# mmbajo/PROBA-V

Measured on AMD Instinct MI355X. Metric: LR-patches/sec fwd+bwd (WDSR-B r12 t9, 16x16, bs128), higher is better.
Workload: dtype f32 (products as 3 scaled-fp16-piece MFMA products, f32 accumulate)

## Files before the change

### proba-v_amd/csrc/kernels_cw4.hip

```cpp
#include "kernels_x6.h"
#include "x6_device.h"
#include <cstdlib>
#include <algorithm>

namespace probav {
#ifdef CW4_DIAG
namespace diag {
#endif

struct Cw4Args {
    ConvGeom g;
    int Wp, Wt, nsplit, SR, nstrips, nslot;
    unsigned mTo, mNvr, mTi, mNslot;
};

namespace {
__device__ __forceinline__ int qdiv(int v, int d, unsigned m) { return (int)__umulhi((unsigned)v, m) + (d == 1 ? v : 0); }
unsigned qmagic(int d) { return d <= 1 ? 0u : (unsigned)((0x100000000ull + (unsigned)d - 1) / (unsigned)d); }
typedef float f32x4u __attribute__((ext_vector_type(4), aligned(4)));
typedef unsigned u32x4b __attribute__((ext_vector_type(4)));
constexpr int CW4_PSE = 151;
constexpr int CW4_PS = 16 * CW4_PSE;
constexpr int CW4_ROW = 8 * CW4_PS;
constexpr unsigned CW4_OOB = 0x40000000u;
}

#ifdef CW4_STAMP
__device__ unsigned long long g_cw4_stamps[1024 * 8];
#endif

#define CW4_SBAR() __builtin_amdgcn_sched_barrier(0)
#ifdef CW4_STAMP
#define CW4_ST(k) do { unsigned long long t_; asm volatile("s_memtime %0\n\ts_waitcnt lgkmcnt(0)" : "=s"(t_) :: "memory"); st_acc[k] += t_ - st_prev; st_prev = t_; } while (0)
#ifdef CW4_STAMP_ROUNDS
#define CW4_STR(k) CW4_ST(k)
#else
#define CW4_STR(k) do { } while (0)
#endif
#else
#define CW4_STR(k) do { } while (0)
#define CW4_ST(k) do { } while (0)
#endif

template <int CIN, int COUT, int TP, bool RELU, bool SKIP, bool BIAS>
__global__ __launch_bounds__(256, 1) void conv3_w4_kernel(Cw4Args a, const float* __restrict__ x, const uint4* __restrict__ wfrag, const float* __restrict__ bias,
                                                         const float* __restrict__ skip, float* __restrict__ y, Amax am)
{
    extern __shared__ __attribute__((aligned(16))) unsigned char lds[];
    constexpr int NST = CIN == 25 ? 5 : 6, KB = 9 * NST, G = 3 * KB;
    constexpr int NW1R = CIN == 25 ? 12 : 8;
    constexpr int NCH = CIN == 25 ? 3 : 4;
    constexpr int PS = CW4_PS, ROW = CW4_ROW;
    constexpr int PD = 2;
    constexpr int TO = TP - 2;
    const ConvGeom& g = a.g;
    const int tid = threadIdx.x, lane = tid & 63, half = lane >> 5, col = lane & 31;
    const int wave = __builtin_amdgcn_readfirstlane(tid >> 6);
    const int per = a.nstrips * a.nsplit;
    const int n = blockIdx.x / per, srem = blockIdx.x - n * per;
    const int strip = srem / a.nsplit, sp = srem - strip * a.nsplit;
    const int ws0 = sp * a.Wt, hb = strip * a.SR;
    const int SRr = g.Ho - hb < a.SR ? g.Ho - hb : a.SR;
    const int nvr = a.Wt * g.To, NV = SRr * nvr, NTL = (NV + 31) >> 5, nround = (NTL + 3) >> 2;
    const int NS = a.nslot;
    float omax = 0.f;
#ifdef CW4_STAMP
    unsigned long long st_t0 = __builtin_amdgcn_s_memtime(), st_r0 = __builtin_amdgcn_s_memrealtime();
    unsigned long long st_prev = st_t0, st_acc[8] = {0, 0, 0, 0, 0, 0, 0, 0};
#endif

    const int lw0 = a.nsplit == 1 ? g.pw : 0, Wl = a.nsplit == 1 ? g.Wi : a.Wt + 2;
    const int nvs = Wl * g.Ti, items = nvs * NCH;
    const int ea = h3_exp(am.x[n]);
    const float sa = pow2i(ea);
    int s_srcb[2], s_offb[2];
    float s_sc[2];
    int s3_o[3], s3_offb = 0;
    float s3_sc[3] = {0.f, 0.f, 0.f};
    {
        auto locate = [&](int lv, int& lw, int& t, int& iwc, int& colok) {
            const int lwr = qdiv(lv, g.Ti, a.mTi);
            t = lv - lwr * g.Ti; lw = lw0 + lwr;
            const int iw = ws0 + lw - g.pw;
            colok = (iw >= 0 ? 1 : 0) & (iw < g.Wi ? 1 : 0);
            iwc = iw < 0 ? 0 : (iw < g.Wi ? iw : g.Wi - 1);
        };
#pragma unroll
        for (int k = 0; k < 2; ++k) {
            const int it = tid + 256 * k;
            const int ic = it < items ? it : items - 1;
            const int lv = CIN == 25 ? (int)(((unsigned)ic * 43691u) >> 17) : ic >> 2;
            const int cc = ic - lv * NCH;
            int lw, t, iwc, colok;
            locate(lv, lw, t, iwc, colok);
            s_srcb[k] = ((iwc * g.Ti + t) * CIN + 8 * cc) * 4;
            s_offb[k] = (lw * TO + t) * 16 + cc * PS;
            s_sc[k] = colok ? sa : 0.f;
        }
        if constexpr (CIN == 25) {
            const int lv = tid < nvs ? tid : nvs - 1;
            int lw, t, iwc, colok;
            locate(lv, lw, t, iwc, colok);
            const int base = ((iwc * g.Ti + t) * CIN + 24) * 4;
            s3_offb = (lw * TO + t) * 16 + 3 * PS;
            const int ok3[3] = {colok && t - 1 >= 0, colok, colok && t + 1 < g.Ti};
#pragma unroll
            for (int j = 0; j < 3; ++j) { s3_o[j] = base + (ok3[j] ? (j - 1) * CIN * 4 : 0); s3_sc[j] = ok3[j] ? sa : 0.f; }
        }
    }
    const long xsample = (long)g.Hi * g.Wi * g.Ti * CIN;
    const __amdgpu_buffer_rsrc_t xrs = __builtin_amdgcn_make_buffer_rsrc(const_cast<float*>(x + (long)n * xsample), 0, (unsigned)xsample * 4u, 0x00020000);
    const int xrowb = g.Wi * g.Ti * CIN * 4;
    struct Staged { u32x4b v[2][2]; unsigned g3[3]; };
    auto row_of = [&](int q, int& rowoff, float& rokf) {
        const int ih = hb - g.ph + q;
        const bool rok = ih >= 0 && ih < g.Hi;
        rowoff = (rok ? ih : 0) * xrowb;
        rokf = rok ? 1.f : 0.f;
    };
    auto stage_load_items = [&](int rowoff, Staged& sv) {
#pragma unroll
        for (int k = 0; k < 2; ++k) {
            sv.v[k][0] = __builtin_amdgcn_raw_buffer_load_b128(xrs, s_srcb[k], rowoff, 0);
            sv.v[k][1] = __builtin_amdgcn_raw_buffer_load_b128(xrs, s_srcb[k] + 16, rowoff, 0);
        }
    };
    auto stage_load_g3 = [&](int rowoff, Staged& sv) {
#ifdef CW4_ABL_NOG3
        sv.g3[0] = sv.g3[1] = sv.g3[2] = 0u; return;
#endif
        if constexpr (CIN == 25) {
#pragma unroll
            for (int j = 0; j < 3; ++j) sv.g3[j] = __builtin_amdgcn_raw_buffer_load_b32(xrs, s3_o[j], rowoff, 0);
        }
    };
    auto slot_of = [&](int q) -> int { return (q - qdiv(q, NS, a.mNslot) * NS) * ROW; };
    struct Cut { float sc[2], sg[3]; f32x2 t[4]; unsigned h0[4], h1[4]; float u[3]; };
    constexpr int ROW_MOPS = CIN == 25 ? 52 : 41;
    auto stage_mop = [&](int m, int slot, float rokf, Staged& sv, Cut& c, bool reload, int rel) {
        if (m < 5) {
            if (m < 2) c.sc[m] = s_sc[m] * rokf;
            else if (CIN == 25) c.sg[m - 2] = s3_sc[m - 2] * rokf;
            return;
        }
        m -= 5;
        if (m < 36) {
            const int k = m / 18, i = m % 18;
            if (i < 16) {
                const int p = i >> 2, op = i & 3;
                if (op == 0) {
                    const u32x4b q = sv.v[k][p >> 1];
                    const f32x2 v = {__uint_as_float(q[2 * (p & 1)]), __uint_as_float(q[2 * (p & 1) + 1])};
                    c.t[p] = v * (f32x2){c.sc[k], c.sc[k]};
                    if (p == 3 && reload) {
                        sv.v[k][0] = __builtin_amdgcn_raw_buffer_load_b128(xrs, s_srcb[k], rel, 0);
                        sv.v[k][1] = __builtin_amdgcn_raw_buffer_load_b128(xrs, s_srcb[k] + 16, rel, 0);
                    }
                } else if (op == 1) {
                    c.h0[p] = __builtin_bit_cast(unsigned, __builtin_convertvector(c.t[p], f16x2));
                } else if (op == 2) {
                    asm("v_fma_mixlo_f16 %0, %1, -1.0, %2 op_sel:[0,0,0] op_sel_hi:[1,0,0]" : "=v"(c.h1[p]) : "v"(c.h0[p]), "v"(c.t[p][0]));
                } else {
                    asm("v_fma_mixhi_f16 %0, %1, -1.0, %2 op_sel:[1,0,0] op_sel_hi:[1,0,0]" : "+v"(c.h1[p]) : "v"(c.h0[p]), "v"(c.t[p][1]));
                }
            } else {
#ifdef CW4_ABL_NOWRITE
                asm volatile("" :: "v"(c.h0[0]), "v"(c.h0[1]), "v"(c.h0[2]), "v"(c.h0[3]), "v"(c.h1[0]), "v"(c.h1[1]), "v"(c.h1[2]), "v"(c.h1[3]));
                return;
#endif
                unsigned char* ent = lds + slot + s_offb[k];
                if (i == 16) *reinterpret_cast<uint4*>(ent) = make_uint4(c.h0[0], c.h0[1], c.h0[2], c.h0[3]);
                else *reinterpret_cast<uint4*>(ent + 4 * PS) = make_uint4(c.h1[0], c.h1[1], c.h1[2], c.h1[3]);
            }
            return;
        }
        if constexpr (CIN == 25) {
            m -= 36;
            if (m < 3) { c.u[m] = __uint_as_float(sv.g3[m]) * c.sg[m]; if (m == 2 && reload) stage_load_g3(rel, sv); }
            else if (m == 3) c.h0[0] = __builtin_bit_cast(unsigned, __builtin_convertvector((f32x2){c.u[0], c.u[1]}, f16x2));
            else if (m == 4) c.h0[1] = __builtin_bit_cast(unsigned, __builtin_convertvector((f32x2){c.u[2], 0.f}, f16x2));
            else if (m == 5) asm("v_fma_mixlo_f16 %0, %1, -1.0, %2 op_sel:[0,0,0] op_sel_hi:[1,0,0]" : "=v"(c.h1[0]) : "v"(c.h0[0]), "v"(c.u[0]));
            else if (m == 6) asm("v_fma_mixhi_f16 %0, %1, -1.0, %2 op_sel:[1,0,0] op_sel_hi:[1,0,0]" : "+v"(c.h1[0]) : "v"(c.h0[0]), "v"(c.u[1]));
            else if (m == 7) c.h1[1] = 0u;
            else if (m == 8) asm("v_fma_mixlo_f16 %0, %1, -1.0, %2 op_sel:[0,0,0] op_sel_hi:[1,0,0]" : "+v"(c.h1[1]) : "v"(c.h0[1]), "v"(c.u[2]));
            else if (m == 9) *reinterpret_cast<uint2*>(lds + slot + s3_offb) = make_uint2(c.h0[0], c.h0[1]);
            else *reinterpret_cast<uint2*>(lds + slot + s3_offb + 4 * PS) = make_uint2(c.h1[0], c.h1[1]);
        }
    };
    auto need = [&](int r) -> int {
        const int vlast = (r + 1) * 128 - 1 < NV - 1 ? (r + 1) * 128 - 1 : NV - 1;
        return qdiv(vlast, nvr, a.mNvr) + 2;
    };

    CW4_ST(3);
    int hiq = nround > 0 ? need(0) : -1;
    Staged p0[4];
    int p0_slot[4];
    float p0_rok[4];
#pragma unroll
    for (int q = 0; q < 4; ++q) {
        int rowoff;
        row_of(q <= hiq ? q : 0, rowoff, p0_rok[q]);
        p0_slot[q] = slot_of(q <= hiq ? q : 0);
        stage_load_items(rowoff, p0[q]);
        stage_load_g3(rowoff, p0[q]);
    }
    constexpr int NQ = ((KB - NW1R) * 64 + 255) / 256;
    u32x4b w1q[NQ];
    const u32x4b* wfrag4 = reinterpret_cast<const u32x4b*>(wfrag);
    const int Z0c = a.Wp * (TP - 2);
    constexpr int NF = KB + NW1R, NF4 = (NF + 3) / 4;
    u32x4b xq[NF4];
#pragma unroll
    for (int i = 0; i < NF4; ++i) {
        int f = 4 * i + wave;
        f = f < NF ? f : NF - 1;
        xq[i] = wfrag4[(f < KB ? 2 * f : 2 * (f - KB) + 1) * 64 + lane];
    }
    const int tab = NS * ROW + (KB - NW1R) * 1024;
    const int tc = tid < g.Cout ? tid : 0;
    const unsigned tew = am.w[tc];
    const float tbv = (bias ? bias : reinterpret_cast<const float*>(am.w))[tc];
#pragma unroll
    for (int i = 0; i < NQ; ++i) {
        int e = tid + 256 * i;
        e = e < (KB - NW1R) * 64 ? e : (KB - NW1R) * 64 - 1;
        w1q[i] = wfrag4[(2 * (NW1R + (e >> 6)) + 1) * 64 + (e & 63)];
    }
    CW4_ST(4);
    if (tid < 32) {
        const int e = -(ea + h3_exp_w(tew));
        reinterpret_cast<int*>(lds + tab)[tid] = e;
        reinterpret_cast<float*>(lds + tab + 128)[tid] = (BIAS && bias && tid < g.Cout) ? ldexpf(tbv, -e) : 0.f;
    }
#pragma unroll
    for (int i = 0; i < NF4; ++i) {
        int f = 4 * i + wave;
        f = f < NF ? f : NF - 1;
        *reinterpret_cast<u32x4b*>(lds + f * 1024 + lane * 16) = xq[i];
    }
    asm volatile("s_waitcnt lgkmcnt(0)\n\ts_barrier" ::: "memory");
    f16x8 w0[KB], w1r[NW1R > 0 ? NW1R : 1];
#pragma unroll
    for (int K = 0; K < KB; ++K) { Frag f; f.u = *reinterpret_cast<const uint4*>(lds + K * 1024 + lane * 16); w0[K] = f.h; }
#pragma unroll
    for (int K = 0; K < NW1R; ++K) { Frag f; f.u = *reinterpret_cast<const uint4*>(lds + (KB + K) * 1024 + lane * 16); w1r[K] = f.h; }
#pragma unroll
    for (int K = 0; K < KB; ++K) asm volatile("" : "+a"(w0[K]));
#pragma unroll
    for (int K = 0; K < NW1R; ++K) asm volatile("" : "+a"(w1r[K]));
    asm volatile("s_waitcnt lgkmcnt(0)\n\ts_barrier" ::: "memory");
    if (a.nsplit == 1) {
        uint4* z = reinterpret_cast<uint4*>(lds);
        for (int i = tid; i < NS * ROW / 16; i += 256) z[i] = make_uint4(0u, 0u, 0u, 0u);
    } else {
        const int nzone = CW4_PSE - Z0c, nplanes = NS * 8;
        for (int i = tid; i < nzone * nplanes; i += 256) {
            const int pl = i / nzone, e = i - pl * nzone;
            *reinterpret_cast<uint4*>(lds + pl * PS + (Z0c + e) * 16) = make_uint4(0u, 0u, 0u, 0u);
        }
        if constexpr (CIN == 25) {
            for (int i = tid; i < Z0c * NS * 2; i += 256) {
                const int pl = i / Z0c, e = i - pl * Z0c;
                *reinterpret_cast<uint4*>(lds + (pl >> 1) * ROW + (3 + 4 * (pl & 1)) * PS + e * 16) = make_uint4(0u, 0u, 0u, 0u);
            }
        }
    }
    asm volatile("s_waitcnt lgkmcnt(0)\n\ts_barrier" ::: "memory");
    CW4_ST(5);
#pragma unroll
    for (int q = 0; q < 4; ++q) {
        Cut c;
#pragma unroll
        for (int m = 0; m < ROW_MOPS; ++m) stage_mop(m, p0_slot[q], p0_rok[q], p0[q], c, false, 0);
    }
    CW4_ST(6);
    const int w1a = NS * ROW + lane * 16;
#pragma unroll
    for (int i = 0; i < NQ; ++i) {
        int e = tid + 256 * i;
        e = e < (KB - NW1R) * 64 ? e : (KB - NW1R) * 64 - 1;
        *reinterpret_cast<u32x4b*>(lds + NS * ROW + e * 16) = w1q[i];
    }
    int eun[16];
    f32x16 bias16;
#pragma unroll
    for (int jj = 0; jj < 4; ++jj) {
        const int4 e4 = *reinterpret_cast<const int4*>(lds + tab + (8 * jj + 4 * half) * 4);
        const float4 b4 = *reinterpret_cast<const float4*>(lds + tab + 128 + (8 * jj + 4 * half) * 4);
        eun[4 * jj] = e4.x; eun[4 * jj + 1] = e4.y; eun[4 * jj + 2] = e4.z; eun[4 * jj + 3] = e4.w;
        bias16[4 * jj] = b4.x; bias16[4 * jj + 1] = b4.y; bias16[4 * jj + 2] = b4.z; bias16[4 * jj + 3] = b4.w;
    }
    const float lo = g.relu ? 0.f : -__builtin_inff();
    (void)lo;
    if (BIAS) asm volatile("" : "+a"(bias16));
    CW4_ST(7);
    asm volatile("s_waitcnt lgkmcnt(0)\n\ts_barrier" ::: "memory");

    const long out_base = ((long)n * g.Ho + hb) * g.Wo * g.To;
    const unsigned ybytes = (unsigned)(SRr * g.Wo * g.To * g.Cout) * 4u;
    const __amdgpu_buffer_rsrc_t yrs = __builtin_amdgcn_make_buffer_rsrc(y + out_base * g.Cout, 0, ybytes, 0x00020000);
    const __amdgpu_buffer_rsrc_t srs = __builtin_amdgcn_make_buffer_rsrc(const_cast<float*>(skip ? skip + out_base * g.Cout : y), 0, skip ? ybytes : 0u, 0x00020000);
    unsigned cofs[4];
#pragma unroll
    for (int jj = 0; jj < 4; ++jj) cofs[jj] = 8 * jj + 4 * half < COUT ? 4u * (8 * jj + 4 * half) : CW4_OOB;

    int offH[5];
    {
        const int pA[5] = {0, 2, 1, 0, 2}, pB[5] = {1, 0, 2, 1, 3};
#pragma unroll
        for (int st = 0; st < 5; ++st) offH[st] = (half ? pB[st] : pA[st]) * PS;
    }
    const int Z0 = a.Wp * TO;
    struct TileTmp { int vi, hrel, rem, w, t, x, e0, s0, s1, s2, b0, b1, b2, dlo, dhi; unsigned yo; };
    constexpr int TILE_STEPS = 14;
    auto tile_step = [&](int step, int tile, TileTmp& q, int (&bs)[9], unsigned (&eo)[4]) {
#define CW4_PIN(v) asm volatile("" : "+v"(v))
        if (step == 0) { const int v = tile * 32 + col; q.vi = v < NV ? v : NV - 1; q.yo = v < NV ? 0u : CW4_OOB; CW4_PIN(q.vi); CW4_PIN(q.yo); }
        if (step == 1) { q.hrel = (int)__umulhi((unsigned)q.vi, a.mNvr); q.rem = q.vi - q.hrel * nvr; CW4_PIN(q.hrel); CW4_PIN(q.rem); }
        if (step == 2) { q.w = (int)__umulhi((unsigned)q.rem, a.mTo); q.t = q.rem - q.w * g.To; CW4_PIN(q.w); CW4_PIN(q.t); }
        if (step == 3) { q.x = q.w * TO + q.t; q.s0 = q.hrel - (int)__umulhi((unsigned)q.hrel, a.mNslot) * NS; CW4_PIN(q.x); CW4_PIN(q.s0); }
        if (step == 4) { q.s1 = q.s0 + 1 < NS ? q.s0 + 1 : q.s0 + 1 - NS; q.e0 = q.x * 16 + (CIN == 32 ? half * PS : 0); CW4_PIN(q.s1); CW4_PIN(q.e0); }
        if (step == 5) { q.s2 = q.s1 + 1 < NS ? q.s1 + 1 : q.s1 + 1 - NS; CW4_PIN(q.s2); }
        if (step == 6) { q.b0 = q.s0 * ROW + q.e0; q.b1 = q.s1 * ROW + q.e0; q.b2 = q.s2 * ROW + q.e0; bs[1] = q.b0; bs[4] = q.b1; bs[7] = q.b2; CW4_PIN(bs[1]); CW4_PIN(bs[4]); CW4_PIN(bs[7]); }
        if (step == 7) { const int z = ((q.x - 1 - Z0) & 15) + Z0 - q.x; q.dlo = q.t == 0 ? z * 16 : -16; CW4_PIN(q.dlo); }
        if (step == 8) { const int z = ((q.x + 1 - Z0) & 15) + Z0 - q.x; q.dhi = q.t == TO - 1 ? z * 16 : 16; CW4_PIN(q.dhi); }
        if (step == 9) { bs[0] = q.b0 + q.dlo; bs[3] = q.b1 + q.dlo; bs[6] = q.b2 + q.dlo; CW4_PIN(bs[0]); CW4_PIN(bs[3]); CW4_PIN(bs[6]); }
        if (step == 10) { bs[2] = q.b0 + q.dhi; bs[5] = q.b1 + q.dhi; bs[8] = q.b2 + q.dhi; CW4_PIN(bs[2]); CW4_PIN(bs[5]); CW4_PIN(bs[8]); }
        if (step == 11) { q.yo += (unsigned)(((q.hrel * g.Wo + ws0 + q.w) * g.To + q.t) * COUT) * 4u; CW4_PIN(q.yo); }
        if (step == 12) { eo[0] = q.yo + cofs[0]; eo[1] = q.yo + cofs[1]; CW4_PIN(eo[0]); CW4_PIN(eo[1]); }
        if (step == 13) { eo[2] = q.yo + cofs[2]; eo[3] = q.yo + cofs[3]; CW4_PIN(eo[2]); CW4_PIN(eo[3]); }
#undef CW4_PIN
    };
    int adr5[5] = {0, 0, 0, 0, 0};
    auto read_A = [&](const int (&bs)[9], int K, Frag (&af)[2]) {
        const int gg = K / NST, st = K % NST, dh = gg / 3, dw = gg % 3;
        if constexpr (CIN == 25) {
            if (dw == 0) {
                const int bm = bs[3 * dh], bz = bs[3 * dh + 1], bp = bs[3 * dh + 2];
                const int b = st == 0 ? bm : st == 1 ? (half ? bz : bm) : st == 2 ? bz : st == 3 ? bp : (half ? bz : bp);
                adr5[st] = b + offH[st];
            }
            const unsigned char* p = lds + adr5[st];
            af[0].u = *reinterpret_cast<const uint4*>(p + dw * TO * 16);
            af[1].u = *reinterpret_cast<const uint4*>(p + dw * TO * 16 + 4 * PS);
        } else {
            const int d = st >> 1, kb = st & 1;
            const unsigned char* p = lds + bs[3 * dh + d];
            af[0].u = *reinterpret_cast<const uint4*>(p + dw * TO * 16 + 2 * kb * PS);
            af[1].u = *reinterpret_cast<const uint4*>(p + dw * TO * 16 + 2 * kb * PS + 4 * PS);
        }
    };
    auto read_W1 = [&](int K, Frag& wf) {
        if (K >= NW1R) wf.u = *reinterpret_cast<const uint4*>(lds + w1a + (K - NW1R) * 1024);
    };

    CW4_ST(2);
    f32x16 accA, accB;
#pragma unroll
    for (int i = 0; i < 16; ++i) { accA[i] = 0.f; accB[i] = 0.f; }
#ifdef CW4_ABL_2ACC
    f32x16 acc2;
    for (int i = 0; i < 16; ++i) acc2[i] = 0.f;
#endif
    f32x4u skq[4];
#pragma unroll
    for (int jj = 0; jj < 4; ++jj) skq[jj] = (f32x4u){0.f, 0.f, 0.f, 0.f};
    int bs[9];
    unsigned eo[4], eo_prev[4] = {CW4_OOB, CW4_OOB, CW4_OOB, CW4_OOB};
    {
        TileTmp q;
#pragma unroll
        for (int st = 0; st < TILE_STEPS; ++st) tile_step(st, wave, q, bs, eo);
    }
    Frag A[PD + 1][2], W1[PD + 1];
#pragma unroll
    for (int K = 0; K < PD; ++K) { read_A(bs, K, A[K]); read_W1(K, W1[K]); }

    Staged sv[2];
    auto round = [&](int r, f32x16& acc, f32x16& pacc) __attribute__((always_inline)) {
        const int hi_next = r + 1 < nround ? need(r + 1) : hiq;
        const int hi_nn = r + 2 < nround ? need(r + 2) : hi_next;
        const int q0 = hiq + 1, q1 = hi_next - hiq >= 2 ? hiq + 2 : hiq + 1;
        const int n0 = hi_next + 1, n1 = hi_nn - hi_next >= 2 ? hi_next + 2 : hi_next + 1;
        int rowoff[2], slot[2];
        float rokf[2], rokn;
        int dummy;
        row_of(q0, dummy, rokf[0]); row_of(q1, dummy, rokf[1]);
        row_of(n0, rowoff[0], rokn); row_of(n1, rowoff[1], rokn);
        slot[0] = slot_of(q0); slot[1] = slot_of(q1);
        Cut cut;
        TileTmp tq;
        int nbs[9];
        unsigned neo[4];
        float m2 = 0.f;
#pragma unroll
        for (int K = 0; K < KB; ++K) {
#pragma unroll
            for (int j = 0; j < 3; ++j) {
                const int gp = 3 * K + j;
                const int sl = K % (PD + 1);
                {
                    f16x8 wa;
                    if (j == 1) { if (K < NW1R) wa = w1r[K < NW1R ? K : 0]; else wa = W1[sl].h; }
                    else wa = w0[K];
                    const f16x8 xb = (j == 0) ? A[sl][1].h : A[sl][0].h;
                    if (gp == 0) {
                        if (BIAS) acc = __builtin_amdgcn_mfma_f32_32x32x16_f16(wa, xb, bias16, 0, 0, 0);
                        else {
                            f32x16 zero;
#pragma unroll
                            for (int i = 0; i < 16; ++i) zero[i] = 0.f;
                            acc = __builtin_amdgcn_mfma_f32_32x32x16_f16(wa, xb, zero, 0, 0, 0);
                        }
                    } else acc = __builtin_amdgcn_mfma_f32_32x32x16_f16(wa, xb, acc, 0, 0, 0);
                }
                CW4_SBAR();
#ifndef CW4_ABL_NOREAD
                if (j == 0) {
                    const int KN = K + PD, sn = KN % (PD + 1);
#ifndef CW4_ABL_W1LATE
                    read_W1(KN < KB ? KN : KN - KB, W1[sn]);
#endif
                    if (KN < KB) read_A(bs, KN, A[sn]); else read_A(nbs, KN - KB, A[sn]);
                }
#ifdef CW4_ABL_W1LATE
                if (j == 1) {
                    const int KN = K + PD, sn = KN % (PD + 1);
                    read_W1(KN < KB ? KN : KN - KB, W1[sn]);
                }
#endif
#endif
                if (K >= 1 && K <= 10 && j == 1) tile_step(K - 1, 4 * (r + 1) + wave, tq, nbs, neo);
                if (K >= 12 && K <= 15 && j == 1) tile_step(K - 2, 4 * (r + 1) + wave, tq, nbs, neo);
                if (K == 11 && j == 1) { CW4_STR(3); asm volatile("s_barrier" ::: "memory"); CW4_STR(4); }
#ifndef CW4_ABL_NOEPI
                if (K < 16 && j == 2) {
                    const int e = K, jj = e >> 2, i = e & 3;
                    float v = ldexpf(pacc[e], eun[e]);
                    if (RELU) v = relu_keep_nan(v, lo);
                    const float o = SKIP ? v + skq[jj][i] : v;
                    skq[jj][i] = o;
                    if ((e & 1) == 0) m2 = o; else asm volatile("v_max3_f32 %0, %0, |%1|, |%2|" : "+v"(omax) : "v"(m2), "v"(o));
                }
                if (j == 1 && (K == 4 || K == 8 || K == 12 || K == 16)) {
                    const int jj = K / 4 - 1;
                    const u32x4b o = {__float_as_uint(skq[jj][0]), __float_as_uint(skq[jj][1]), __float_as_uint(skq[jj][2]), __float_as_uint(skq[jj][3])};
                    if (COUT == 32 || jj < 3) __builtin_amdgcn_raw_buffer_store_b128(o, yrs, eo_prev[jj], 0, 0);
                    else __builtin_amdgcn_raw_buffer_store_b32(o[0], yrs, eo_prev[jj], 0, 0);
                    if (K == 16) omax = r == 0 ? 0.f : omax;
                }
                if (SKIP && (K == 17 || K == 18) && j > 0) {
                    const int jj = 2 * (K - 17) + j - 1;
                    if (COUT == 32 || jj < 3) {
                        const u32x4b q = __builtin_amdgcn_raw_buffer_load_b128(srs, eo[jj], 0, 0);
                        skq[jj] = (f32x4u){__uint_as_float(q[0]), __uint_as_float(q[1]), __uint_as_float(q[2]), __uint_as_float(q[3])};
                    } else {
                        const unsigned q = __builtin_amdgcn_raw_buffer_load_b32(srs, eo[jj], 0, 0);
                        skq[jj] = (f32x4u){__uint_as_float(q), 0.f, 0.f, 0.f};
                    }
                }
#endif
#ifndef CW4_ABL_NOSTAGE
                {
                    constexpr int NKS = (2 * ROW_MOPS + 5) / 6, KS0 = KB - PD - NKS;
                    if (K >= KS0 && K < KS0 + NKS && j > 0) {
                        const int m0 = (K - KS0) * 6 + 3 * (j - 1);
#pragma unroll
                        for (int m = m0; m < m0 + 3; ++m)
                            if (m < 2 * ROW_MOPS) {
#ifdef CW4_ABL_NOCUT
                                if (m == 0) asm volatile("" :: "v"(sv[0].v[0][0]), "v"(sv[0].v[1][1]), "v"(sv[1].v[0][0]), "v"(sv[1].v[1][1]));
                                continue;
#endif
                                stage_mop(m % ROW_MOPS, slot[m / ROW_MOPS], rokf[m / ROW_MOPS], sv[m / ROW_MOPS], cut, true, rowoff[m / ROW_MOPS]);
                            }
                    }
                }
#endif
                CW4_SBAR();
            }
        }
        CW4_STR(5);
#pragma unroll
        for (int d = 0; d < 9; ++d) bs[d] = nbs[d];
#pragma unroll
        for (int jj = 0; jj < 4; ++jj) { eo_prev[jj] = eo[jj]; eo[jj] = neo[jj]; }
        hiq = hi_next;
    };
    {
        const int hi1 = 1 < nround ? need(1) : hiq;
        const int n0 = hiq + 1, n1 = hi1 - hiq >= 2 ? hiq + 2 : hiq + 1;
        int ro;
        float rk;
        row_of(n0, ro, rk); stage_load_items(ro, sv[0]); stage_load_g3(ro, sv[0]);
        row_of(n1, ro, rk); stage_load_items(ro, sv[1]); stage_load_g3(ro, sv[1]);
    }
#pragma unroll 1
    for (int r = 0; r < nround; r += 2) {
        round(r, accA, accB);
        round(r + 1, accB, accA);
    }
    {
#pragma unroll
        for (int e = 0; e < 16; ++e) {
            const int jj = e >> 2, i = e & 3;
            float v = ldexpf(accB[e], eun[e]);
            if (RELU) v = relu_keep_nan(v, lo);
            const float o = SKIP ? v + skq[jj][i] : v;
            skq[jj][i] = o;
            omax = fmaxf(omax, fabsf(o));
        }
        if (nround == 0) omax = 0.f;
#pragma unroll
        for (int jj = 0; jj < 4; ++jj) {
            const u32x4b o = {__float_as_uint(skq[jj][0]), __float_as_uint(skq[jj][1]), __float_as_uint(skq[jj][2]), __float_as_uint(skq[jj][3])};
            if (COUT == 32 || jj < 3) __builtin_amdgcn_raw_buffer_store_b128(o, yrs, eo_prev[jj], 0, 0);
            else __builtin_amdgcn_raw_buffer_store_b32(o[0], yrs, eo_prev[jj], 0, 0);
        }
    }
#ifdef CW4_ABL_2ACC
    for (int i = 0; i < 16; ++i) omax += acc2[i];
#endif
    if (am.y) amax_commit(omax, am.y + n);
#ifdef CW4_STAMP
    if (lane == 0 && blockIdx.x < 256) {
        unsigned long long* o = g_cw4_stamps + (blockIdx.x * 4 + wave) * 8;
        o[0] = __builtin_amdgcn_s_memtime() - st_t0; o[1] = __builtin_amdgcn_s_memrealtime() - st_r0;
        for (int k = 2; k < 8; ++k) o[k] = st_acc[k];
    }
#endif
}

static bool cw4_plan(const ConvGeom& g, Cw4Args& p, size_t& lds_bytes, int& grid)
{
    if (g.kh != 3 || g.kw != 3 || g.kt != 3 || g.reflect_hw || g.reflect_t) return false;
    if (!((g.Cin == 25 && g.Cout == 32) || (g.Cin == 32 && (g.Cout == 25 || g.Cout == 32)))) return false;
    if (g.ph != 1 || g.pw != 1 || g.pt != 1) return false;
    if (g.Ho != g.Hi || g.Wo != g.Wi || g.To != g.Ti) return false;
    if (g.To != 9 && g.To != 7) return false;
    if (g.Ho < 3) return false;
    const int Tp = g.To + 2;
    for (int ns = 1; ns <= 4; ++ns) {
        if (g.Wo % ns) continue;
        const int wt = g.Wo / ns, nvr = wt * g.To;
        const int wp = wt + 2;
        const int nvs = (ns == 1 ? g.Wi : wt + 2) * g.Ti, items = nvs * (g.Cin == 25 ? 3 : 4);
        if (items > 512 || nvs > 256 || nvr < 64 || wp * g.To + 16 + 2 * g.To > CW4_PSE) continue;
        int nstrips = (256 + g.N * ns - 1) / (g.N * ns);
        if (nstrips < 1) nstrips = 1;
        if (nstrips > g.Ho / 4) nstrips = g.Ho / 4 > 0 ? g.Ho / 4 : 1;
        const int SR = (g.Ho + nstrips - 1) / nstrips;
        nstrips = (g.Ho + SR - 1) / SR;
        const int NV = SR * nvr, nround = ((NV + 31) / 32 + 3) / 4;
        auto needf = [&](int r) { const int vl = std::min(NV - 1, (r + 1) * 128 - 1); return vl / nvr + 2; };
        int nslot = needf(0) + 1;
        for (int r = 0; r + 1 < nround; ++r) nslot = std::max(nslot, needf(r + 1) - (r * 128) / nvr + 1);
        const int kb = g.Cin == 25 ? 45 : 54, nw1r = g.Cin == 25 ? 12 : 8;
        const size_t need = (size_t)nslot * CW4_ROW + (size_t)(kb - nw1r) * 1024 + 256;
        if (need > 163840) continue;
        p.g = g; p.Wp = wp; p.Wt = wt; p.nsplit = ns; p.SR = SR; p.nstrips = nstrips; p.nslot = nslot;
        p.mTo = qmagic(g.To); p.mNvr = qmagic(nvr); p.mTi = qmagic(g.Ti); p.mNslot = qmagic(nslot);
        lds_bytes = need; grid = g.N * nstrips * ns;
        return true;
    }
    return false;
}

bool cw4_conv_supported(const ConvGeom& g, bool gated)
{
    Cw4Args p;
    size_t lds_bytes;
    int grid;
    return !gated && cw4_plan(g, p, lds_bytes, grid);
}

bool cw4_conv_plan_ints(const ConvGeom& g, bool gated, int out[5])
{
    Cw4Args p;
    size_t lds_bytes;
    int grid;
    if (gated || !cw4_plan(g, p, lds_bytes, grid)) return false;
    out[0] = p.nsplit; out[1] = p.nstrips; out[2] = p.SR; out[3] = p.nslot; out[4] = grid;
    return true;
}

int cw4_conv_forward(const ConvGeom& g, const float* x, const float* wfrag, const float* bias, const float* skip, float* y, const Amax& am, hipStream_t s)
{
    Cw4Args p;
    size_t lds_bytes;
    int grid;
    if (!cw4_plan(g, p, lds_bytes, grid)) { set_error("cw4_conv_forward: unsupported geometry", hipSuccess); return PROBAV_EINVAL; }
    if (!am.x || !am.w) { set_error("cw4_conv_forward: H3 arithmetic needs the operands' amax slots", hipSuccess); return PROBAV_EINVAL; }
#define CW4_LAUNCH(C, O, T, R, S, B) return launch_lds<conv3_w4_kernel<C, O, T, R, S, B>>("conv3_w4", dim3(grid), dim3(256), lds_bytes, s, p, x, (const uint4*)wfrag, bias, skip, y, am)
#define CW4_LAUNCH_T(C, O) do { if (g.To == 9) CW4_LAUNCH(C, O, 11, true, true, true); else CW4_LAUNCH(C, O, 9, true, true, true); } while (0)
    if (g.Cin == 25 && g.To == 9 && !g.relu && skip && bias) CW4_LAUNCH(25, 32, 11, false, true, true);
    else if (g.Cin == 32 && g.Cout == 25 && g.To == 9 && !g.relu && !skip && !bias) CW4_LAUNCH(32, 25, 11, false, false, false);
    else if (g.Cin == 25) CW4_LAUNCH_T(25, 32);
    else if (g.Cout == 25) CW4_LAUNCH_T(32, 25);
    else CW4_LAUNCH_T(32, 32);
#undef CW4_LAUNCH_T
#undef CW4_LAUNCH
}

#ifdef CW4_DIAG
}
#endif
}
```

Baseline: 20620.

## Split leftover tail tiles' K reduction across waves in conv3 w4 kernel

When the last strip leaves one or two 32-voxel tiles beyond a multiple of four, those tiles are pulled out of the main round loop. They get a dedicated tail phase where the four waves split the K chain of MFMAs and reduce the partial accumulators through LDS. The aim is to stop a final round running with most waves idle on clamped, masked tiles. The cost is extra barriers, LDS exchange traffic and a duplicated epilogue, plus odd-round handling in the main loop.

```diff
diff --git a/proba-v_amd/csrc/kernels_cw4.hip b/proba-v_amd/csrc/kernels_cw4.hip
--- a/proba-v_amd/csrc/kernels_cw4.hip
+++ b/proba-v_amd/csrc/kernels_cw4.hip
@@ -2,6 +2,7 @@
 #include "x6_device.h"
 #include <cstdlib>
 #include <algorithm>
+#include <type_traits>
 
 namespace probav {
 #ifdef CW4_DIAG
@@ -61,7 +62,12 @@
     const int strip = srem / a.nsplit, sp = srem - strip * a.nsplit;
     const int ws0 = sp * a.Wt, hb = strip * a.SR;
     const int SRr = g.Ho - hb < a.SR ? g.Ho - hb : a.SR;
-    const int nvr = a.Wt * g.To, NV = SRr * nvr, NTL = (NV + 31) >> 5, nround = (NTL + 3) >> 2;
+    const int nvr = a.Wt * g.To, NV = SRr * nvr;
+    const int NVS = g.Ho * nvr, NTLS = (NVS + 31) >> 5;
+    const int ntail = (hb + SRr == g.Ho && ((NTLS & 3) == 1 || (NTLS & 3) == 2)) ? (NTLS & 3) : 0;
+    const int NVm = ntail ? NV - (NVS - 32 * (NTLS - ntail)) : NV;
+    const int NTL = (NVm + 31) >> 5, nmain = (NTL + 3) >> 2, nround = nmain + (ntail ? 1 : 0);
+    const int NVml = NVm > 0 ? NVm - 1 : 0;
     const int NS = a.nslot;
     float omax = 0.f;
 #ifdef CW4_STAMP
@@ -188,7 +194,7 @@
         }
     };
     auto need = [&](int r) -> int {
-        const int vlast = (r + 1) * 128 - 1 < NV - 1 ? (r + 1) * 128 - 1 : NV - 1;
+        const int vlast = r >= nmain ? NV - 1 : ((r + 1) * 128 - 1 < NVml ? (r + 1) * 128 - 1 : NVml);
         return qdiv(vlast, nvr, a.mNvr) + 2;
     };
 
@@ -314,9 +320,9 @@
     const int Z0 = a.Wp * TO;
     struct TileTmp { int vi, hrel, rem, w, t, x, e0, s0, s1, s2, b0, b1, b2, dlo, dhi; unsigned yo; };
     constexpr int TILE_STEPS = 14;
-    auto tile_step = [&](int step, int tile, TileTmp& q, int (&bs)[9], unsigned (&eo)[4]) {
+    auto tile_step = [&](int step, int vbase, int vend, int vclamp, TileTmp& q, int (&bs)[9], unsigned (&eo)[4]) {
 #define CW4_PIN(v) asm volatile("" : "+v"(v))
-        if (step == 0) { const int v = tile * 32 + col; q.vi = v < NV ? v : NV - 1; q.yo = v < NV ? 0u : CW4_OOB; CW4_PIN(q.vi); CW4_PIN(q.yo); }
+        if (step == 0) { const int v = vbase + col; q.vi = v < vend ? v : vclamp; q.yo = v < vend ? 0u : CW4_OOB; CW4_PIN(q.vi); CW4_PIN(q.yo); }
         if (step == 1) { q.hrel = (int)__umulhi((unsigned)q.vi, a.mNvr); q.rem = q.vi - q.hrel * nvr; CW4_PIN(q.hrel); CW4_PIN(q.rem); }
         if (step == 2) { q.w = (int)__umulhi((unsigned)q.rem, a.mTo); q.t = q.rem - q.w * g.To; CW4_PIN(q.w); CW4_PIN(q.t); }
         if (step == 3) { q.x = q.w * TO + q.t; q.s0 = q.hrel - (int)__umulhi((unsigned)q.hrel, a.mNslot) * NS; CW4_PIN(q.x); CW4_PIN(q.s0); }
@@ -371,7 +377,7 @@
     {
         TileTmp q;
 #pragma unroll
-        for (int st = 0; st < TILE_STEPS; ++st) tile_step(st, wave, q, bs, eo);
+        for (int st = 0; st < TILE_STEPS; ++st) tile_step(st, 32 * wave, NVm, NVml, q, bs, eo);
     }
     Frag A[PD + 1][2], W1[PD + 1];
 #pragma unroll
@@ -431,8 +437,8 @@
                 }
 #endif
 #endif
-                if (K >= 1 && K <= 10 && j == 1) tile_step(K - 1, 4 * (r + 1) + wave, tq, nbs, neo);
-                if (K >= 12 && K <= 15 && j == 1) tile_step(K - 2, 4 * (r + 1) + wave, tq, nbs, neo);
+                if (K >= 1 && K <= 10 && j == 1) tile_step(K - 1, 128 * (r + 1) + 32 * wave, NVm, NVml, tq, nbs, neo);
+                if (K >= 12 && K <= 15 && j == 1) tile_step(K - 2, 128 * (r + 1) + 32 * wave, NVm, NVml, tq, nbs, neo);
                 if (K == 11 && j == 1) { CW4_STR(3); asm volatile("s_barrier" ::: "memory"); CW4_STR(4); }
 #ifndef CW4_ABL_NOEPI
                 if (K < 16 && j == 2) {
@@ -496,8 +502,10 @@
         row_of(n0, ro, rk); stage_load_items(ro, sv[0]); stage_load_g3(ro, sv[0]);
         row_of(n1, ro, rk); stage_load_items(ro, sv[1]); stage_load_g3(ro, sv[1]);
     }
+    const int rodd = nmain & 1;
+    if (rodd) round(0, accB, accA);
 #pragma unroll 1
-    for (int r = 0; r < nround; r += 2) {
+    for (int r = rodd; r < nmain; r += 2) {
         round(r, accA, accB);
         round(r + 1, accB, accA);
     }
@@ -511,12 +519,102 @@
             skq[jj][i] = o;
             omax = fmaxf(omax, fabsf(o));
         }
-        if (nround == 0) omax = 0.f;
+        if (nmain == 0) omax = 0.f;
 #pragma unroll
         for (int jj = 0; jj < 4; ++jj) {
             const u32x4b o = {__float_as_uint(skq[jj][0]), __float_as_uint(skq[jj][1]), __float_as_uint(skq[jj][2]), __float_as_uint(skq[jj][3])};
             if (COUT == 32 || jj < 3) __builtin_amdgcn_raw_buffer_store_b128(o, yrs, eo_prev[jj], 0, 0);
             else __builtin_amdgcn_raw_buffer_store_b32(o[0], yrs, eo_prev[jj], 0, 0);
+        }
+    }
+    if (ntail) {
+        const int tt = ntail == 1 ? 0 : wave >> 1;
+        const bool lead = ntail == 1 ? wave == 0 : (wave & 1) == 0;
+        int tbs[9];
+        unsigned teo[4];
+        {
+            TileTmp q;
+#pragma unroll
+            for (int st = 0; st < TILE_STEPS; ++st) tile_step(st, NVm + 32 * tt, NV, NV - 1, q, tbs, teo);
+        }
+        asm volatile("s_waitcnt lgkmcnt(0)\n\ts_barrier" ::: "memory");
+        f32x16 tacc;
+#pragma unroll
+        for (int i = 0; i < 16; ++i) tacc[i] = 0.f;
+        auto chain = [&](auto k0, auto k1) __attribute__((always_inline)) {
+            constexpr int K0 = decltype(k0)::value, K1 = decltype(k1)::value;
+#pragma unroll
+            for (int K = K0; K < K1; ++K) {
+                const int gg = K / NST, st = K % NST, dh = gg / 3, dw = gg % 3;
+                Frag af[2], wf;
+                if constexpr (CIN == 25) {
+                    const int bm = tbs[3 * dh], bz = tbs[3 * dh + 1], bp = tbs[3 * dh + 2];
+                    const int b = st == 0 ? bm : st == 1 ? (half ? bz : bm) : st == 2 ? bz : st == 3 ? bp : (half ? bz : bp);
+                    const unsigned char* p = lds + b + offH[st] + dw * TO * 16;
+                    af[0].u = *reinterpret_cast<const uint4*>(p);
+                    af[1].u = *reinterpret_cast<const uint4*>(p + 4 * PS);
+                } else {
+                    const unsigned char* p = lds + tbs[3 * dh + (st >> 1)] + dw * TO * 16 + 2 * (st & 1) * PS;
+                    af[0].u = *reinterpret_cast<const uint4*>(p);
+                    af[1].u = *reinterpret_cast<const uint4*>(p + 4 * PS);
+                }
+                if (K >= NW1R) wf.u = *reinterpret_cast<const uint4*>(lds + w1a + (K - NW1R) * 1024);
+                else wf.h = w1r[K < NW1R ? K : 0];
+                if (K == 0 && BIAS) tacc = __builtin_amdgcn_mfma_f32_32x32x16_f16(w0[K], af[1].h, bias16, 0, 0, 0);
+                else tacc = __builtin_amdgcn_mfma_f32_32x32x16_f16(w0[K], af[1].h, tacc, 0, 0, 0);
+                tacc = __builtin_amdgcn_mfma_f32_32x32x16_f16(wf.h, af[0].h, tacc, 0, 0, 0);
+                tacc = __builtin_amdgcn_mfma_f32_32x32x16_f16(w0[K], af[0].h, tacc, 0, 0, 0);
+            }
+        };
+        using std::integral_constant;
+        if (ntail == 1) {
+            if (wave == 0) chain(integral_constant<int, 0>{}, integral_constant<int, KB / 4>{});
+            else if (wave == 1) chain(integral_constant<int, KB / 4>{}, integral_constant<int, KB / 2>{});
+            else if (wave == 2) chain(integral_constant<int, KB / 2>{}, integral_constant<int, 3 * KB / 4>{});
+            else chain(integral_constant<int, 3 * KB / 4>{}, integral_constant<int, KB>{});
+        } else {
+            if ((wave & 1) == 0) chain(integral_constant<int, 0>{}, integral_constant<int, KB / 2>{});
+            else chain(integral_constant<int, KB / 2>{}, integral_constant<int, KB>{});
+        }
+        asm volatile("s_waitcnt lgkmcnt(0)\n\ts_barrier" ::: "memory");
+        float* xch = reinterpret_cast<float*>(lds) + wave * 1024 + lane * 4;
+        if (!lead) {
+#pragma unroll
+            for (int jj = 0; jj < 4; ++jj) *reinterpret_cast<float4*>(xch + jj * 256) = make_float4(tacc[4 * jj], tacc[4 * jj + 1], tacc[4 * jj + 2], tacc[4 * jj + 3]);
+        }
+        asm volatile("s_waitcnt lgkmcnt(0)\n\ts_barrier" ::: "memory");
+        if (lead) {
+            const int nadd = ntail == 1 ? 3 : 1;
+            for (int c = 1; c <= nadd; ++c) {
+#pragma unroll
+                for (int jj = 0; jj < 4; ++jj) {
+                    const float4 p = *reinterpret_cast<const float4*>(xch + c * 1024 + jj * 256);
+                    tacc[4 * jj] += p.x; tacc[4 * jj + 1] += p.y; tacc[4 * jj + 2] += p.z; tacc[4 * jj + 3] += p.w;
+                }
+            }
+            float tmax = 0.f;
+#pragma unroll
+            for (int jj = 0; jj < 4; ++jj) {
+                f32x4u sk = {0.f, 0.f, 0.f, 0.f};
+                if (SKIP) {
+                    if (COUT == 32 || jj < 3) {
+                        const u32x4b q = __builtin_amdgcn_raw_buffer_load_b128(srs, teo[jj], 0, 0);
+                        sk = (f32x4u){__uint_as_float(q[0]), __uint_as_float(q[1]), __uint_as_float(q[2]), __uint_as_float(q[3])};
+                    } else sk[0] = __uint_as_float(__builtin_amdgcn_raw_buffer_load_b32(srs, teo[jj], 0, 0));
+                }
+                u32x4b o;
+#pragma unroll
+                for (int i = 0; i < 4; ++i) {
+                    float v = ldexpf(tacc[4 * jj + i], eun[4 * jj + i]);
+                    if (RELU) v = relu_keep_nan(v, lo);
+                    const float ov = SKIP ? v + sk[i] : v;
+                    tmax = fmaxf(tmax, fabsf(ov));
+                    o[i] = __float_as_uint(ov);
+                }
+                if (COUT == 32 || jj < 3) __builtin_amdgcn_raw_buffer_store_b128(o, yrs, teo[jj], 0, 0);
+                else __builtin_amdgcn_raw_buffer_store_b32(o[0], yrs, teo[jj], 0, 0);
+            }
+            omax = fmaxf(omax, tmax);
         }
     }
 #ifdef CW4_ABL_2ACC
```

After: 20670 (median of 6 runs). About the same (+0.2%).
